# kaegi/adaptive-sph

Hardware: AMD Instinct MI355X
Metric: particle-steps/sec (whole node), 2D dam-break N=1M DFSPH; 1/2/4/8 GPUs (higher is better)
Workload: dtype f32; 1 GPU; dam_break_1m: 2D dam-break, 1024x1024 = 1 048 576 uniform-h particles, HybridDFSPH; particles=1048576, solver=HybridDFSPH, parallelism=single GPU

## Files before the change

adaptive_sph_amd/csrc/sph_api.hip:

```cpp
#include <hip/hip_runtime.h>

#include <algorithm>
#include <chrono>
#include <cmath>
#include <cstdarg>
#include <cstdio>
#include <cstdlib>
#include <cstring>
#include <string>
#include <vector>

#include "sph_context.hpp"
#include "sph_lambda.hpp"

int Profiler::find(const char* name)
{
    for (size_t i = 0; i < recs.size(); i++)
        if (recs[i].name == name) return (int)i;
    recs.push_back(Rec{name, 0, 0, {}});
    return (int)recs.size() - 1;
}
bool Profiler::wants(const char* name) const
{
    return mode == 1 || mode == 3 || mode == 4 || (mode == 2 && (step_index & 7u) == 0u && strncmp(name, "density", 7) == 0);
// ... 181 lines not shown
        for (int k = 1; k < 4; k++) {
            r.min_x = fminf(r.min_x, s[k].min_x); r.min_y = fminf(r.min_y, s[k].min_y);
            r.max_x = fmaxf(r.max_x, s[k].max_x); r.max_y = fmaxf(r.max_y, s[k].max_y);
            r.h_max = fmaxf(r.h_max, s[k].h_max); r.h_min = fminf(r.h_min, s[k].h_min);
            r.min_cfl = fminf(r.min_cfl, s[k].min_cfl);
        }
        r.pad = seq - 1u;
        *out = r;
        if (seq) {
            __threadfence_system();
            ((volatile HeaderOut*)out)->pad = seq;
        }
    }
}

__global__ __launch_bounds__(1024) void k_header_ahead(const HeaderOut* __restrict__ partials, uint32_t nparts, const SolverCtrl* __restrict__ ctrl,
                                                       HeaderOut* __restrict__ out, const DeviceStatus* __restrict__ status, SolverCtrl* __restrict__ h_ctrl,
                                                       DeviceStatus* __restrict__ h_status, uint32_t seq)
{
    if (ctrl->done == 0u) {
        if (h_ctrl && threadIdx.x == 0) {
            SolverCtrl v = *ctrl;
            v.seq = seq - 1u;
            *h_ctrl = v;
            *h_status = *status;
            __threadfence_system();
            ((volatile SolverCtrl*)h_ctrl)->seq = seq;
        }
        return;
    }
    const float INF = __uint_as_float(0x7f800000u);
    HeaderOut o{INF, INF, -INF, -INF, 0.f, INF, INF, 0};
    for (uint32_t k0 = threadIdx.x; k0 < nparts; k0 += 4096u) {
        HeaderOut q[4];
#pragma unroll
        for (uint32_t u = 0; u < 4u; u++) q[u] = partials[min(k0 + 1024u * u, nparts - 1u)];
#pragma unroll
        for (uint32_t u = 0; u < 4u; u++) {
            o.min_x = fminf(o.min_x, q[u].min_x); o.min_y = fminf(o.min_y, q[u].min_y);
            o.max_x = fmaxf(o.max_x, q[u].max_x); o.max_y = fmaxf(o.max_y, q[u].max_y);
            o.h_max = fmaxf(o.h_max, q[u].h_max); o.h_min = fminf(o.h_min, q[u].h_min);
            o.min_cfl = fminf(o.min_cfl, q[u].min_cfl);
        }
    }
    o.min_x = wave_min(o.min_x); o.min_y = wave_min(o.min_y); o.max_x = wave_max(o.max_x); o.max_y = wave_max(o.max_y);
    o.h_max = wave_max(o.h_max); o.h_min = wave_min(o.h_min); o.min_cfl = wave_min(o.min_cfl);
    __shared__ HeaderOut s[16];
    const int lane = threadIdx.x & 63, w = threadIdx.x >> 6;
    if (lane == 0) s[w] = o;
    __syncthreads();
    if (threadIdx.x == 0) {
        HeaderOut r = s[0];
        for (int k = 1; k < 16; k++) {
            r.min_x = fminf(r.min_x, s[k].min_x); r.min_y = fminf(r.min_y, s[k].min_y);
            r.max_x = fmaxf(r.max_x, s[k].max_x); r.max_y = fmaxf(r.max_y, s[k].max_y);
            r.h_max = fmaxf(r.h_max, s[k].h_max); r.h_min = fminf(r.h_min, s[k].h_min);
            r.min_cfl = fminf(r.min_cfl, s[k].min_cfl);
        }
        *out = r;
        if (h_ctrl) {
            SolverCtrl v = *ctrl;
            v.seq = seq - 1u;
            *h_ctrl = v;
            *h_status = *status;
            __threadfence_system();
            ((volatile SolverCtrl*)h_ctrl)->seq = seq;
        }
    }
}

__global__ __launch_bounds__(256) void k_pack_upload(uint32_t n, const float* __restrict__ mass, const float2* __restrict__ pos,
                                                      const float2* __restrict__ velin, float4* __restrict__ pm, float2* __restrict__ vel,
                                                      uint32_t* __restrict__ orig, float* __restrict__ lvl, float* __restrict__ lvlold,
                                                      float* __restrict__ h2_next)
{
    uint32_t i = blockIdx.x * 256 + threadIdx.x;
    if (i >= n) return;
    float2 p = pos[i];
    pm[i] = make_float4(p.x, p.y, mass[i], 0.f);
    h2_next[i] = h_from_mass(mass[i], 1.f);
    vel[i] = velin[i];
    orig[i] = i;
    lvl[i] = __uint_as_float(0x7fc00000u);
    lvlold[i] = 0.f;
// ... 193 lines not shown
    o.chain = num("SPH_CHAIN", -1);
    o.accel_generic = flag("SPH_ACCEL_GENERIC");
    o.jacobi_generic = flag("SPH_JACOBI_GENERIC");
    o.source_generic = flag("SPH_SOURCE_GENERIC");
    o.slab_general = flag("SPH_SLAB_GENERAL");
    o.slab_level_plain = flag("SPH_SLAB_LEVEL_PLAIN");
    o.level_serial = flag("SPH_LEVEL_SERIAL");
    o.level_batch8 = flag("SPH_LEVEL_BATCH8");
    o.level_queue = num("SPH_LEVEL_QUEUE", 1) != 0 ? 1 : 0;
    o.offset_lists = num("SPH_OFFSET_LISTS", 1) != 0 ? 1 : 0;
    o.no_fuse = flag("SPH_NO_FUSE");
    o.side_stream_normal = flag("SPH_SIDE_STREAM_NORMAL");
    o.tile = num("SPH_TILE", 0);
    o.ahead_build = num("SPH_AHEAD_BUILD", 1) != 0 ? 1 : 0;
    o.inc_sort = num("SPH_INC_SORT", 1);
    o.slab_paced = num("SPH_SLAB_PACED", 1) != 0 ? 1 : 0;
    o.slab_records = num("SPH_SLAB_RECORDS", 1) != 0 ? 1 : 0;
    o.side_cus = num("SPH_SIDE_CUS", 0);
    o.main_exclude = num("SPH_MAIN_EXCLUDE", 0) != 0 ? 1 : 0;
    o.ipc_fuse_max_bytes = std::max(num("SPH_IPC_FUSE_MAX_BYTES", 64 << 10), 0);
    o.ipc_copy_min_bytes = std::max(num("SPH_IPC_COPY_MIN_BYTES", 256 << 10), 0);
#else
    static const char* const lab_only[] = {"SPH_PACED", "SPH_PACE_LEAD", "SPH_PACE_PRED", "SPH_CHAIN", "SPH_ACCEL_GENERIC", "SPH_JACOBI_GENERIC", "SPH_SOURCE_GENERIC",
                                           "SPH_SLAB_GENERAL", "SPH_SLAB_LEVEL_PLAIN", "SPH_LEVEL_SERIAL", "SPH_LEVEL_BATCH8", "SPH_LEVEL_QUEUE", "SPH_OFFSET_LISTS",
                                           "SPH_NO_FUSE", "SPH_SIDE_STREAM_NORMAL", "SPH_TILE", "SPH_AHEAD_BUILD", "SPH_INC_SORT", "SPH_SLAB_PACED", "SPH_SLAB_RECORDS",
                                           "SPH_SIDE_CUS", "SPH_MAIN_EXCLUDE", "SPH_IPC_FUSE_MAX_BYTES", "SPH_IPC_COPY_MIN_BYTES"};
    static bool warned = false;
    if (!warned)
        for (const char* name : lab_only)
            if (getenv(name)) {
                fprintf(stderr, "libsph_hip: %s is a laboratory switch and is IGNORED by the product library (use SPH_HIP_LIBRARY=libsph_lab.so, scripts/README.md)\n", name);
                warned = true;
            }
#endif
    return o;
}

extern "C" int sph_create(uint64_t n_capacity, int device_id, const sph_plane* planes, int n_planes, sph_ctx** out)
{
    if (!out || n_planes < 0 || n_planes > SPH_MAX_PLANES || (n_planes > 0 && !planes)) return SPH_ERR_INVALID_ARGUMENT;
// ... 96 lines not shown
}

extern "C" void sph_destroy(sph_ctx* c)
{
    if (!c) return;
    (void)hipSetDevice(c->device);
    if (c->stream) (void)hipStreamSynchronize(c->stream);
    if (c->stream2) (void)hipStreamSynchronize(c->stream2);
    dist_release(c);
    DevBuf* all[] = {&c->pm[0], &c->pm[1], &c->vel[0], &c->vel[1], &c->orig[0], &c->orig[1], &c->lvl[0], &c->lvl[1], &c->lvlold[0],
                     &c->lvlold[1], &c->vel_tmp, &c->key[0], &c->key[1], &c->val[0], &c->val[1], &c->sort_scratch, &c->cxy, &c->cell_start,
                     &c->cs_scratch, &c->hdr_ahead_partials, &c->h2n[0], &c->h2n[1], &c->lam_prev, &c->nl, &c->nlx, &c->tile_raw, &c->tile_h, &c->tile_h_ext, &c->lvl_changed_d, &c->lvl_tmp, &c->lvl_nrm, &c->lvl_state, &c->lvl_when, &c->lvl_mark, &c->lvl_queue, &c->nloff, &c->nlh, &c->flag_surface,
                     &c->flag_insufficient, &c->con_thr, &c->con_consumed, &c->con_h, &c->flag_reduced, &c->szc[0], &c->szc[1], &c->omega, &c->stash, &c->nl_ext, &c->nlx_ext, &c->nl_ok, &c->mrho, &c->pt0, &c->pt1, &c->prec0, &c->prec1, &c->xv, &c->rho, &c->lam_sum, &c->lam_grad, &c->wall_pl, &c->wall_cnt, &c->constf, &c->aii, &c->src, &c->p0, &c->p1, &c->pacc, &c->dens_err,
                     &c->stat, &c->ncount, &c->planes_d, &c->lam_lut, &c->dlam_lut, &c->hdr_partials, &c->hdr_out, &c->ctrl, &c->status,
                     &c->n_tiles, &c->red_partials, &c->scratch, &c->split_patterns, &c->akey[0], &c->akey[1], &c->aval[0], &c->aval[1], &c->acxy, &c->acell_start, &c->pm2,
                     &c->atile_raw, &c->atile_h, &c->inc_head, &c->inc_next, &c->inc_bsum, &c->inc_movers, &c->export_d_off, &c->export_d_idx,
                     &c->cand_rec, &c->cand_cls, &c->cand_cnt, &c->cand_off, &c->cand_idx, &c->cand_scan, &c->cand_red, &c->rnd_rec, &c->rnd_keys, &c->rnd_out, &c->rnd_max, &c->rnd_prev};
    for (auto b : all) b->release();
    if (c->hdr_host) (void)hipHostFree(c->hdr_host);
    if (c->ctrl_host) (void)hipHostFree(c->ctrl_host);
    if (c->status_host) (void)hipHostFree(c->status_host);
    if (c->lvl_changed) (void)hipHostFree(c->lvl_changed);
    for (auto& e : c->ev)
        if (e) (void)hipEventDestroy(e);
    if (c->ev_sync) (void)hipEventDestroy(c->ev_sync);
    if (c->stream) (void)hipStreamDestroy(c->stream);
    if (c->stream2) (void)hipStreamDestroy(c->stream2);
    if (c->ev_fork) (void)hipEventDestroy(c->ev_fork);
    delete c;
}

// ... 814 lines not shown
    int nb = (int)((n + 255) / 256);
    if (nb > HDR_BLOCKS) nb = HDR_BLOCKS;
    if (nb < 1) nb = 1;
    hipLaunchKernelGGL(k_header, dim3(nb), dim3(256), 0, s, c->pm[c->pcur].as<float4>(), c->vel[c->cur].as<float2>(), n, rest_density, from_mass,
                       c->h2n[c->cur].as<float>(), c->hdr_partials.as<HeaderOut>(), owned);
    c->publish_seq++;
    if (c->publish_seq == 0u) c->publish_seq = 1u;
    const bool mapped = out_dev == c->hdr_host_dev;
    hipLaunchKernelGGL(k_header_final, dim3(1), dim3(256), 0, s, c->hdr_partials.as<HeaderOut>(), nb, out_dev, mapped ? c->publish_seq : 0u);
    if (mapped) {
        c->hint_word = &((volatile HeaderOut*)c->hdr_host)->pad;
        c->hint_seq = c->publish_seq;
    }
}

void launch_header_ahead(sph_ctx* c, uint32_t nblocks, HeaderOut* out_dev, bool publish)
{
    ProfScope ps(&c->prof, "header_ahead", c->stream);
    uint32_t seq = 0;
    if (publish) {
        c->publish_seq++;
        if (c->publish_seq == 0u) c->publish_seq = 1u;
        seq = c->publish_seq;
        c->publish_folded = true;
    }
    hipLaunchKernelGGL(k_header_ahead, dim3(1), dim3(1024), 0, c->stream, c->hdr_ahead_partials.as<HeaderOut>(), nblocks, c->ctrl.as<SolverCtrl>(), out_dev,
                       c->status.as<DeviceStatus>(), publish ? c->ctrl_host_dev : (SolverCtrl*)nullptr, publish ? c->status_host_dev : (DeviceStatus*)nullptr, seq);
}

void launch_publish(sph_ctx* c)
{
    if (c->publish_folded) {
        c->publish_folded = false;
        return;
    }
    c->publish_seq++;
    if (c->publish_seq == 0u) c->publish_seq = 1u;
    hipLaunchKernelGGL(k_publish, dim3(1), dim3(64), 0, c->stream, c->ctrl.as<SolverCtrl>(), c->status.as<DeviceStatus>(), c->ctrl_host_dev,
                       c->status_host_dev, c->publish_seq);
}

void launch_check_neighborhood(sph_ctx* c, const SweepArgs& a)
// ... 5 lines not shown
```

adaptive_sph_amd/csrc/sph_context.hpp:

```cpp
#pragma once

#include <hip/hip_runtime.h>

#include <chrono>
#include <cstdarg>
#include <cstdio>
#include <string>
#include <vector>

#include "sph_internal.hpp"

struct DevBuf {
    void* p = nullptr;
    size_t bytes = 0;
    hipError_t ensure(size_t need)
    {
        if (need <= bytes) return hipSuccess;
        if (p) (void)hipFree(p);
        p = nullptr;
        bytes = 0;
        size_t grow = need + need / 4 + 256;
        hipError_t e = hipMalloc(&p, grow);
        if (e == hipSuccess) bytes = grow;
        return e;
// ... 3 lines not shown
        if (p) (void)hipFree(p);
        p = nullptr;
        bytes = 0;
    }
    template <class T>
    T* as() const { return (T*)p; }
};

struct TmpBuf : DevBuf {
    TmpBuf() = default;
    TmpBuf(const TmpBuf&) = delete;
    TmpBuf& operator=(const TmpBuf&) = delete;
    ~TmpBuf() { release(); }
};

struct Options {
    int exact = 0;
    int paced = 1;
    int pace_lead = 0;
    int pace_pred = 0xffff;
    int chain = -1;
    int overlap = -1;
    int accel_generic = 0;
    int jacobi_generic = 0;
    int source_generic = 0;
    int slab_general = 0;
    int slab_level_plain = 0;
    int level_serial = 0;
    int level_batch8 = 0;
    int offset_lists = 1;
    int level_queue = 1;
// ... 108 lines not shown
        int rebalance_every = 0;
        DevBuf hist;
        uint32_t rebalances = 0;
        uint64_t stat_exchanges = 0, stat_bytes_sent = 0, stat_bytes_recv = 0, stat_allreduces = 0, stat_step0 = 0;
    } dist;

    GridP grid{};
    bool grid_valid = false;
    GridP fgrid{};
    int tile_ts = 0, tile_tsx = 0, tile_tsy = 0;
    DevBuf tile_raw, tile_h, tile_h_ext, nlx;
    DevBuf nloff, nlh;
    DevBuf akey[2], aval[2], acxy, acell_start, pm2;
    DevBuf atile_raw, atile_h;
    DevBuf inc_head, inc_next, inc_bsum, inc_movers;
    uint32_t inc_epoch = 0;
    int inc_radix_streak = 0;
    bool inc_count_valid = false;
    struct Ahead {
        bool valid = false;
        GridP g{};
        float h_max = 0.f, h_min = 0.f, rest_density = 0.f;
        int tile_ts = 0, tile_tsx = 0, tile_tsy = 0;
        uint64_t n = 0;
    } ahead;
    DevBuf hdr_ahead_partials;
    bool hdr_ahead = false;
    float hdr_ahead_rest_density = 0.f;
    DevBuf h2n[2];
    DevBuf lam_prev;
// ... 57 lines not shown
```

adaptive_sph_amd/csrc/sph_internal.hpp:

```cpp
#pragma once

#include <hip/hip_runtime.h>
#include <hip/hip_ext.h>
#include <stdint.h>

#include <string>
#include <vector>

#include "sph_device.h"
#include "sph_ffi.h"

struct Profiler {
    int mode = 0;
    uint64_t step_index = 0;
    struct Rec {
        std::string name;
        uint64_t launches = 0;
        double total_ms = 0;
        std::vector<float> samples;
    };
    struct Pending {
        int rec;
        hipEvent_t a, b;
        int slot;
// ... 47 lines not shown
    uint32_t done;
    uint32_t iters;
    uint32_t cur;
    uint32_t peer_error;
    uint32_t normal, singular, negative;
    float sum_err, max_err;
    uint32_t slot_done[2];
    uint32_t seq;
};

struct DeviceStatus {
    uint32_t error;
    uint32_t info;
};

struct CellKeyGen {
    const float4* pm;
    GridP g;
    const uint8_t* gone;
    uint32_t n_gone, gone_from;
    int clamp = 0;
};
int radix_sort_pairs(hipStream_t s, Profiler* prof, uint32_t* keyA, uint32_t* valA, uint32_t* keyB, uint32_t* valB,
                     uint32_t n, int bits, uint32_t* hist_scratch , const CellKeyGen* keygen = nullptr);
size_t radix_sort_scratch_elems(uint32_t n);
struct ReorderIO {
    const float4* pm_in;
    const float2* vel_in;
    const uint32_t* orig_in;
    const float *lvl_in, *lvlold_in;
    float4* pm_out;
    float2* vel_out;
    uint32_t* orig_out;
    float *lvl_out, *lvlold_out;
    uint32_t* cxy_out;
    const float* h2n_in;
    float* h2n_out;
    const float* lam_in;
    float* lam_prev_out;
    const uint8_t* szc_in;
    uint8_t* szc_out;
};
size_t incremental_sort_block_sums(uint32_t ncells);
void incremental_cell_sort_reorder(hipStream_t s, Profiler* prof, uint32_t n, const float4* pm_new, const IncClassifyP& q, bool classified,
                                   const uint32_t* cell_start_cur, uint32_t* key_out, uint32_t* cell_start_out, const ReorderIO& io, uint32_t* bsum, uint32_t* movers,
                                   uint32_t* movers_host);

void incremental_cell_sort_perm(hipStream_t s, Profiler* prof, uint32_t n, uint32_t n_prev, const CellKeyGen& kg, const IncClassifyP& q, const uint32_t* cell_start_cur,
                                uint32_t* key_out, uint32_t* perm_out, uint32_t* cell_start_out, uint32_t* bsum, uint32_t* movers, uint32_t* movers_host);

void launch_reorder(hipStream_t s, Profiler* prof, uint32_t n, GridP g, const uint32_t* sorted_key, const uint32_t* perm,
                    const float4* pm_in, const float2* vel_in, const uint32_t* orig_in, const float* lvl_in,
                    const float* lvlold_in, float4* pm_out, float2* vel_out, uint32_t* orig_out, float* lvl_out,
                    float* lvlold_out, uint32_t* cxy, const float* h2n_in = nullptr, float* h2n_out = nullptr,
                    const float* lam_in = nullptr, float* lam_prev_out = nullptr, void* cell_start_scratch = nullptr,
                    const uint8_t* szc_in = nullptr, uint8_t* szc_out = nullptr);
size_t cell_start_scratch_bytes();
void launch_cell_start(hipStream_t s, Profiler* prof, const uint32_t* sorted_key, uint32_t n, uint32_t ncells,
                       uint32_t* cell_start , void* scratch ,
                       bool count_zeroed = false );
void launch_tile_hmax(hipStream_t s, Profiler* prof, uint32_t n, const float4* pm, GridP g, int ts, int tsx, int tsy, uint32_t* raw,
// ... 124 lines not shown
    int center_diff;
    int plain_propagate;
    const uint8_t* edge;
    int replay_step_lists;
    const float4* pm_cell;
};
void launch_max_disp(hipStream_t s, Profiler* prof, uint32_t n, const float4* pm_old, const float4* pm_new, uint32_t* out);
void launch_tile_redilate(hipStream_t s, Profiler* prof, int tsx, int tsy, int d, const uint32_t* raw, uint32_t* out);
void launch_level_detect(hipStream_t s, Profiler* prof, const SweepArgs& a, const LevelArgs& l);
void launch_level_propagate(hipStream_t s, Profiler* prof, const SweepArgs& a, const LevelArgs& l, uint32_t t, uint32_t* changed);
void launch_fill_stash(hipStream_t s, Profiler* prof, const SweepArgs& a, const LevelArgs& l, float* stash);
void launch_level_smooth(hipStream_t s, Profiler* prof, const SweepArgs& a, const LevelArgs& l, const float4* pm_new, const float* in, float* out);
void launch_classify(hipStream_t s, Profiler* prof, uint32_t n, const float4* pm, const float* level, uint8_t* size_class, const uint8_t* owned,
                     const uint32_t* orig, DeviceStatus* status, const sph_params* p);
void launch_header_ahead(sph_ctx* c, uint32_t nblocks, HeaderOut* out_dev, bool publish = false);
void launch_iisph2_scale(hipStream_t s, Profiler* prof, const SweepArgs& a);
void launch_check_aii(hipStream_t s, Profiler* prof, const SweepArgs& a);
void launch_vel_add_pacc(hipStream_t s, Profiler* prof, const SweepArgs& a);
void launch_integrate(hipStream_t s, Profiler* prof, const SweepArgs& a, float4* pm_out, int mode);

struct EditSrc {
    uint32_t obj;
    uint32_t set_idx;
};
struct EditSet {
    uint32_t fields;
    float mass, px, py, vx, vy, h2, h2_next, lvl, lvlold;
};
struct sph_ctx;
int regather_host_order(sph_ctx* c, uint32_t n_new, const EditSrc* d_src, const EditSet* d_sets);
// ... 2 lines not shown
```

adaptive_sph_amd/csrc/sph_sort.hip:

```cpp
#include "sph_internal.hpp"

#define RS_ITEMS 32
#define RS_TILE (64 * RS_ITEMS)

template <int NB>
__device__ __forceinline__ uint64_t rs_peers(uint32_t d, bool valid)
{
    uint64_t peers = __ballot(valid);
#pragma unroll
    for (int b = 0; b < NB; b++) {
        const bool bit = (d >> b) & 1u;
        const uint64_t m = __ballot(bit);
        peers &= bit ? m : ~m;
    }
    return peers;
}

__device__ __forceinline__ uint32_t cell_key_of(const CellKeyGen& kg, uint32_t i)
{
    if (kg.gone && i < kg.n_gone && kg.gone[i] >= kg.gone_from) return kg.g.ncells;
    const float4 p = kg.pm[i];
    if (kg.clamp) return cell_key_clamped(kg.g, p.x, p.y);
    const int cx = (int)floorf(p.x / kg.g.cs) - kg.g.minx;
    const int cy = (int)floorf(p.y / kg.g.cs) - kg.g.miny;
// ... 291 lines not shown
        if (lane >= o) x += y;
    }
    if (lane == 63) ws[w] = x;
    __syncthreads();
    uint32_t run = base_s + x - own;
    for (int k = 0; k < w; k++) run += ws[k];
#pragma unroll
    for (uint32_t u = 0; u < 4u; u++) {
        if (c0 + u < ncells) cell_start[c0 + u] = run;
        run += v[u];
        if (c0 + u + 1u == ncells) cell_start[ncells] = run;
    }
    if (blockIdx.x == 0 && tid == 0) {
        *movers_host = *movers;
        *movers = 0u;
    }
}

template <bool PERM>
__global__ __launch_bounds__(256) void k_inc_place_reorder(uint32_t n, IncGrid G, const uint32_t* __restrict__ cell_start_cur, const uint32_t* __restrict__ cell_start_nxt,
                                                            const uint32_t* __restrict__ nk, const uint8_t* __restrict__ mv, const uint32_t* __restrict__ next,
                                                            const unsigned long long* __restrict__ head, uint32_t epoch, const uint32_t* __restrict__ cxy_cur,
                                                            uint32_t* __restrict__ key_out, ReorderIO io, uint32_t* __restrict__ perm_out)
{
    const uint32_t i = blockIdx.x * 256 + threadIdx.x;
    if (i >= n) return;
    const uint32_t flag = mv[i];
    if (PERM && flag == 2u) return;
    const uint32_t c = nk[i];
    const bool mover = flag != 0u;
// ... 31 lines not shown
        return;
    }
    io.pm_out[dst] = pm;
    io.vel_out[dst] = vel;
    io.orig_out[dst] = orig;
    io.lvl_out[dst] = lvl;
    io.lvlold_out[dst] = lvlold;
    if (io.h2n_in) io.h2n_out[dst] = io.h2n_in[i];
    if (io.lam_in) io.lam_prev_out[dst] = io.lam_in[i];
    if (io.szc_in) io.szc_out[dst] = io.szc_in[i];
    const uint32_t cy = c / (uint32_t)G.nxt.sx;
    io.cxy_out[dst] = (c - cy * (uint32_t)G.nxt.sx) | (cy << 16);
}

size_t incremental_sort_block_sums(uint32_t ncells) { return ((size_t)ncells + INC_CELLS - 1) / INC_CELLS; }

void incremental_cell_sort_reorder(hipStream_t s, Profiler* prof, uint32_t n, const float4* pm_new, const IncClassifyP& q, bool classified,
                                   const uint32_t* cell_start_cur, uint32_t* key_out, uint32_t* cell_start_out, const ReorderIO& io, uint32_t* bsum, uint32_t* movers,
                                   uint32_t* movers_host)
{
    const IncGrid G{q.cur, q.nxt};
    const uint32_t ncells = q.nxt.ncells, cblocks = (uint32_t)incremental_sort_block_sums(ncells);
    if (!classified) {
        ProfScope ps(prof, "inc_classify", s);
        hipLaunchKernelGGL(k_inc_classify, dim3((n + 255) / 256), dim3(256), 0, s, n, pm_new, q);
    }
    {
        ProfScope ps(prof, "inc_count", s);
        hipLaunchKernelGGL(k_inc_count, dim3(cblocks), dim3(INC_CELLS), 0, s, G, cell_start_cur, q.mv, q.next, q.head, q.epoch, cell_start_out, bsum, movers);
    }
    {
        ProfScope ps(prof, "inc_scan", s);
        hipLaunchKernelGGL(k_inc_scan, dim3(cblocks), dim3(256), 0, s, ncells, cell_start_out, bsum, movers, movers_host);
    }
    {
        ProfScope ps(prof, "inc_reorder", s);
        hipLaunchKernelGGL(k_inc_place_reorder<false>, dim3((n + 255) / 256), dim3(256), 0, s, n, G, cell_start_cur, cell_start_out, q.nk, q.mv, q.next, q.head,
                           q.epoch, q.cxy_cur, key_out, io, (uint32_t*)nullptr);
    }
}

void incremental_cell_sort_perm(hipStream_t s, Profiler* prof, uint32_t n, uint32_t n_prev, const CellKeyGen& kg, const IncClassifyP& q, const uint32_t* cell_start_cur,
                                uint32_t* key_out, uint32_t* perm_out, uint32_t* cell_start_out, uint32_t* bsum, uint32_t* movers, uint32_t* movers_host)
{
    const IncGrid G{q.cur, q.nxt};
    const uint32_t ncells = q.nxt.ncells, cblocks = (uint32_t)incremental_sort_block_sums(ncells);
    {
        ProfScope ps(prof, "inc_classify", s);
// ... 170 lines not shown
```

adaptive_sph_amd/csrc/sph_step.hip:

```cpp
#include <atomic>
#include <hip/hip_runtime.h>
#include <rccl/rccl.h>

#include <array>
#include <cmath>
#include <cstdlib>
#include <cstring>
#include <condition_variable>
#include <functional>
#include <memory>
#include <mutex>
#include <vector>

#include "sph_dist.hpp"

SweepArgs make_args(sph_ctx* c, const StepP& sp)
{
    SweepArgs a{};
    const int k = c->cur;
    a.g = c->fgrid;
    a.sp = sp;
    a.n = c->dist.on ? c->dist.n_tot : (uint32_t)c->n;
    a.exact = c->exact;
    a.cell_start = c->cell_start.as<uint32_t>();
// ... 373 lines not shown
            if (m.n) launch_jacobi_update(m.c->stream, &m.c->prof, m.a, (int)k, q.residual_density, q.max_avg_error, q.max_iters, multi);
        }
        if ((rc = exchange_and_sweep_a(G, M, q, k + 1))) return rc;
    }
    for (auto& m : M) {
        (void)hipSetDevice(m.c->device);
        SolverCtrl* hand_host = handoff ? m.c->ctrl_host_dev + 1 : nullptr;
        uint32_t* gate_out = handoff ? (uint32_t*)(m.c->ctrl.as<SolverCtrl>() + 2) : nullptr;
        if (!m.n || q.tail == 0 ) {
            if (handoff) launch_solver_handoff(m.c->stream, &m.c->prof, m.c->ctrl.as<SolverCtrl>(), hand_host, gate_out);
            continue;
        }
        launch_solver_tail(m.c->stream, &m.c->prof, m.a, q.tail, m.c->pm[m.c->pcur ^ 1].as<float4>(), -1, q.residual_density,
                           q.max_avg_error, q.max_iters, hand_host, gate_out);
        if (q.tail == 1  && source_term_on_records(m.a)) m.a.xv_ok = true;
        if (q.tail >= 2  && m.a.hdr_partials) launch_header_ahead(m.c, (m.n + 255u) / 256u, m.c->hdr_host_dev, publish_next && !multi);
    }
    return SPH_OK;
}
static void solve_stats(Member& m, const SolveQ& q, const SolverCtrl& h)
{
    m.c->pressure_cur = h.cur;
    sph_solver_stats* st = q.density_solver ? &m.st.density_solver : &m.st.div_solver;
    st->iters = h.iters;
    st->converged = 1;
    st->normal_count = h.normal;
    st->singular_count = h.singular;
    st->negative_count = h.negative;
    st->avg_error = h.normal > 0 ? h.sum_err / (float)h.normal : NAN;
    st->max_error = h.max_err;
}
// ... 118 lines not shown
        return c0->fail(SPH_ERR_INVALID_ARGUMENT, "center diff level estimation method needs density values");
    if (!p->level_estimation_after_advection && !p->use_extended_range_for_level_estimation)
        return c0->fail(SPH_ERR_INVALID_ARGUMENT, "assertion failed: simulation_params.use_extended_range_for_level_estimation");
    if (!G.multi() && c0->n == 0) return c0->fail(SPH_ERR_INVALID_ARGUMENT, "called `Option::unwrap()` on a `None` value (no particles)");
    if (!p->level_estimation_after_advection && !(p->level_estimation_range / SPH_ETA >= 2.f))
        return c0->fail(SPH_ERR_UNSUPPORTED, "level_estimation_range / 1.9 = %g < 2: the reference then steps on lists narrower than the SPH support, which this build does not cover",
                        (double)(p->level_estimation_range / SPH_ETA));
    for (auto c : G.m)
        if (c->poisoned) return c->fail(SPH_ERR_POISONED, "an earlier step failed inside the step: the particle state is undefined until sph_upload");
    *started = true;
    const bool no_records = c0->opt.accel_generic != 0;
    const bool paced = c0->opt.paced != 0 && p->max_iters <= 0x7fffu && (!G.multi() || c0->opt.slab_paced != 0);
    for (auto c : G.m) c->paced_step = paced;
    for (auto c : G.m) c->dist.overlap_env = c0->opt.overlap;
    for (auto c : G.m) c->publish_folded = false;

    const bool tev = c0->prof.mode == 1;
    for (auto& m : M) {
        (void)hipSetDevice(m.c->device);
        if (tev) (void)hipEventRecord(m.c->ev[0], m.c->stream);
    }

    std::vector<std::vector<float>> red(M.size(), std::vector<float>(8));
    int hdr_rc = SPH_OK, setup_rc = SPH_OK;
    bool slab_fused = false;
    const float slab_slack_k = (level_on && p->level_estimation_after_advection && G.multi())
                                   ? fmaxf(2.f, c0->h_max_step > 0.f ? 4.f * c0->last_dmax / c0->h_max_step : 0.f) : 0.f;
    const float halo_base_k = fmaxf(4.f, level_on ? p->level_estimation_range / SPH_ETA : 0.f);
    auto header_ready = [&](sph_ctx* c) { return h_from_mass_mode && c->hdr_ahead && c->hdr_ahead_rest_density == p->rest_density; };
    const bool ahead_usable = !G.multi() && header_ready(c0);
// ... 716 lines not shown
            if (!m.n) launch_ctrl_reset(m.c->stream, m.c->ctrl.as<SolverCtrl>(), m.a.gate);
            if (m.n) launch_source_term(m.c->stream, &m.c->prof, m.a, kind, residual_density);
        }
    };
    auto rec = [&](int e) {
        if (tev)
            for (auto& m : M) {
                (void)hipSetDevice(m.c->device);
                (void)hipEventRecord(m.c->ev[e], m.c->stream);
            }
    };
    enum { T_NONE = 0, T_VEL = 1, T_VX = 2, T_HYBRID = 3 };
    g_trace.mark(3);
    struct AheadPlan {
        bool on = false, incremental = false;
        GridP g{};
        int tile_ts = 0, tile_tsx = 0, tile_tsy = 0;
        IncClassifyP q{};
    } plan;
    auto plan_ahead_build = [&]() -> int {
        sph_ctx* c = c0;
        plan = AheadPlan{};
        if (G.multi() || !paced || !c->opt.ahead_build || !h_from_mass_mode || p->constrain_neighborhood_count || (!c->uniform_h && c->tile_ts <= 0) ||
            (c->uniform_h && c->tile_ts != 0) || c->exact || M[0].n == 0)
            return SPH_OK;
        const uint32_t n = M[0].n;
        const float cs = c->fgrid.cs;
        const int ts = c->tile_ts, margin = 2 * (ts > 0 ? ts : 1);
        GridP g{};
        g.cs = cs;
// ... 31 lines not shown
        hipStream_t s = c->stream;
        const size_t head_before = c->inc_head.bytes;
        HIPCHK(c, c->inc_head.ensure((size_t)g.ncells * 8));
        if (c->inc_head.bytes != head_before) HIPCHK(c, hipMemsetAsync(c->inc_head.p, 0, c->inc_head.bytes, s));
        HIPCHK(c, c->inc_next.ensure((size_t)c->cap * 4));
        HIPCHK(c, c->inc_bsum.ensure(incremental_sort_block_sums(g.ncells) * 4));
        if (!c->inc_movers.p) {
            HIPCHK(c, c->inc_movers.ensure(4));
            HIPCHK(c, hipMemsetAsync(c->inc_movers.p, 0, 4, s));
        }
        if (++c->inc_epoch == 0u) c->inc_epoch = 1u;
        plan.incremental = true;
        plan.q = IncClassifyP{c->fgrid, g, c->cxy.as<uint32_t>(), c->akey[1].as<uint32_t>(), c->aval[1].as<uint8_t>(), c->inc_next.as<uint32_t>(),
                              c->inc_head.as<unsigned long long>(), c->inc_epoch};
        M[0].a.inc = plan.q;
        return SPH_OK;
    };
    bool ahead_deferred = level_on;
    const std::function<int()> queue_ahead_build = [&]() -> int {
        sph_ctx* c = c0;
        if (ahead_deferred) return SPH_OK;
        c->ahead.valid = false;
        if (!plan.on) return SPH_OK;
        const uint32_t n = M[0].n;
        const GridP g = plan.g;
        hipStream_t s = c->stream;
        const int k = c->cur;
        const float4* integrated = c->pm[c->pcur ^ 1].as<float4>();
        if (plan.incremental) {
            const ReorderIO io{integrated, c->vel[k].as<float2>(), c->orig[k].as<uint32_t>(), c->lvl[k].as<float>(), c->lvlold[k].as<float>(), c->pm2.as<float4>(),
                               c->vel[k ^ 1].as<float2>(), c->orig[k ^ 1].as<uint32_t>(), c->lvl[k ^ 1].as<float>(), c->lvlold[k ^ 1].as<float>(), c->acxy.as<uint32_t>(),
                               c->h2n[k].as<float>(), c->h2n[k ^ 1].as<float>(),  nullptr, nullptr, c->szc[k].as<uint8_t>(), c->szc[k ^ 1].as<uint8_t>()};
            incremental_cell_sort_reorder(s, &c->prof, n, integrated, plan.q,  true, c->cell_start.as<uint32_t>(), c->akey[0].as<uint32_t>(),
                                          c->acell_start.as<uint32_t>(), io, c->inc_bsum.as<uint32_t>(), c->inc_movers.as<uint32_t>(),
                                          (uint32_t*)(c->ctrl_host_dev + 2) + 1);
            c->inc_count_valid = true;
        } else {
            const CellKeyGen kg{integrated, g, nullptr, 0u, (uint32_t)SC_GONE_FROM, 1};
            const int res = radix_sort_pairs(s, &c->prof, c->akey[0].as<uint32_t>(), c->aval[0].as<uint32_t>(), c->akey[1].as<uint32_t>(), c->aval[1].as<uint32_t>(), n,
                                             ilog2_ceil(g.ncells), c->sort_scratch.as<uint32_t>(), &kg);
            if (res == 1) {
                std::swap(c->akey[0], c->akey[1]);
                std::swap(c->aval[0], c->aval[1]);
            }
            launch_reorder(s, &c->prof, n, g, c->akey[0].as<uint32_t>(), c->aval[0].as<uint32_t>(), integrated, c->vel[k].as<float2>(), c->orig[k].as<uint32_t>(),
                           c->lvl[k].as<float>(), c->lvlold[k].as<float>(), c->pm2.as<float4>(), c->vel[k ^ 1].as<float2>(), c->orig[k ^ 1].as<uint32_t>(),
                           c->lvl[k ^ 1].as<float>(), c->lvlold[k ^ 1].as<float>(), c->acxy.as<uint32_t>(), c->h2n[k].as<float>(), c->h2n[k ^ 1].as<float>(),
                           c->lam_sum.as<float>(), c->lam_prev.as<float>(), c->cs_scratch.p, c->szc[k].as<uint8_t>(), c->szc[k ^ 1].as<uint8_t>());
            launch_cell_start(s, &c->prof, c->akey[0].as<uint32_t>(), n, g.ncells, c->acell_start.as<uint32_t>(), c->cs_scratch.p, true);
        }
// ... 394 lines not shown
```

Before: 2.434 billion particle-steps/s.

## Fuse incremental-sort count and scan with header-ahead reduction into one launch

Replaces the separate inc_count and inc_scan kernels with a single-pass count+scan kernel. It uses ticketed blocks and epoch-tagged decoupled lookback on per-block aggregates. The header_ahead reduction is folded into an extra block of that same launch instead of being its own kernel. This is on by default for uniform-h, single-device, non-level runs, and is meant to cut per-step launch count and serialization gaps. The cost is spin-waiting between blocks, a bounded spin timeout that could silently produce wrong offsets, and more complex state handoff.

```diff
diff --git a/adaptive_sph_amd/csrc/sph_api.hip b/adaptive_sph_amd/csrc/sph_api.hip
--- a/adaptive_sph_amd/csrc/sph_api.hip
+++ b/adaptive_sph_amd/csrc/sph_api.hip
@@ -219,60 +219,7 @@
     }
 }
 
-__global__ __launch_bounds__(1024) void k_header_ahead(const HeaderOut* __restrict__ partials, uint32_t nparts, const SolverCtrl* __restrict__ ctrl,
-                                                       HeaderOut* __restrict__ out, const DeviceStatus* __restrict__ status, SolverCtrl* __restrict__ h_ctrl,
-                                                       DeviceStatus* __restrict__ h_status, uint32_t seq)
-{
-    if (ctrl->done == 0u) {
-        if (h_ctrl && threadIdx.x == 0) {
-            SolverCtrl v = *ctrl;
-            v.seq = seq - 1u;
-            *h_ctrl = v;
-            *h_status = *status;
-            __threadfence_system();
-            ((volatile SolverCtrl*)h_ctrl)->seq = seq;
-        }
-        return;
-    }
-    const float INF = __uint_as_float(0x7f800000u);
-    HeaderOut o{INF, INF, -INF, -INF, 0.f, INF, INF, 0};
-    for (uint32_t k0 = threadIdx.x; k0 < nparts; k0 += 4096u) {
-        HeaderOut q[4];
-#pragma unroll
-        for (uint32_t u = 0; u < 4u; u++) q[u] = partials[min(k0 + 1024u * u, nparts - 1u)];
-#pragma unroll
-        for (uint32_t u = 0; u < 4u; u++) {
-            o.min_x = fminf(o.min_x, q[u].min_x); o.min_y = fminf(o.min_y, q[u].min_y);
-            o.max_x = fmaxf(o.max_x, q[u].max_x); o.max_y = fmaxf(o.max_y, q[u].max_y);
-            o.h_max = fmaxf(o.h_max, q[u].h_max); o.h_min = fminf(o.h_min, q[u].h_min);
-            o.min_cfl = fminf(o.min_cfl, q[u].min_cfl);
-        }
-    }
-    o.min_x = wave_min(o.min_x); o.min_y = wave_min(o.min_y); o.max_x = wave_max(o.max_x); o.max_y = wave_max(o.max_y);
-    o.h_max = wave_max(o.h_max); o.h_min = wave_min(o.h_min); o.min_cfl = wave_min(o.min_cfl);
-    __shared__ HeaderOut s[16];
-    const int lane = threadIdx.x & 63, w = threadIdx.x >> 6;
-    if (lane == 0) s[w] = o;
-    __syncthreads();
-    if (threadIdx.x == 0) {
-        HeaderOut r = s[0];
-        for (int k = 1; k < 16; k++) {
-            r.min_x = fminf(r.min_x, s[k].min_x); r.min_y = fminf(r.min_y, s[k].min_y);
-            r.max_x = fmaxf(r.max_x, s[k].max_x); r.max_y = fmaxf(r.max_y, s[k].max_y);
-            r.h_max = fmaxf(r.h_max, s[k].h_max); r.h_min = fminf(r.h_min, s[k].h_min);
-            r.min_cfl = fminf(r.min_cfl, s[k].min_cfl);
-        }
-        *out = r;
-        if (h_ctrl) {
-            SolverCtrl v = *ctrl;
-            v.seq = seq - 1u;
-            *h_ctrl = v;
-            *h_status = *status;
-            __threadfence_system();
-            ((volatile SolverCtrl*)h_ctrl)->seq = seq;
-        }
-    }
-}
+__global__ __launch_bounds__(1024) void k_header_ahead(HeaderAheadP a) { header_ahead_block(a); }
 
 __global__ __launch_bounds__(256) void k_pack_upload(uint32_t n, const float* __restrict__ mass, const float2* __restrict__ pos,
                                                       const float2* __restrict__ velin, float4* __restrict__ pm, float2* __restrict__ vel,
@@ -496,6 +443,7 @@
     o.tile = num("SPH_TILE", 0);
     o.ahead_build = num("SPH_AHEAD_BUILD", 1) != 0 ? 1 : 0;
     o.inc_sort = num("SPH_INC_SORT", 1);
+    o.fold = num("SPH_FOLD", SPH_FOLD_DEFAULT) & SPH_FOLD_DEFAULT;
     o.slab_paced = num("SPH_SLAB_PACED", 1) != 0 ? 1 : 0;
     o.slab_records = num("SPH_SLAB_RECORDS", 1) != 0 ? 1 : 0;
     o.side_cus = num("SPH_SIDE_CUS", 0);
@@ -505,7 +453,7 @@
 #else
     static const char* const lab_only[] = {"SPH_PACED", "SPH_PACE_LEAD", "SPH_PACE_PRED", "SPH_CHAIN", "SPH_ACCEL_GENERIC", "SPH_JACOBI_GENERIC", "SPH_SOURCE_GENERIC",
                                            "SPH_SLAB_GENERAL", "SPH_SLAB_LEVEL_PLAIN", "SPH_LEVEL_SERIAL", "SPH_LEVEL_BATCH8", "SPH_LEVEL_QUEUE", "SPH_OFFSET_LISTS",
-                                           "SPH_NO_FUSE", "SPH_SIDE_STREAM_NORMAL", "SPH_TILE", "SPH_AHEAD_BUILD", "SPH_INC_SORT", "SPH_SLAB_PACED", "SPH_SLAB_RECORDS",
+                                           "SPH_NO_FUSE", "SPH_SIDE_STREAM_NORMAL", "SPH_TILE", "SPH_AHEAD_BUILD", "SPH_INC_SORT", "SPH_FOLD", "SPH_SLAB_PACED", "SPH_SLAB_RECORDS",
                                            "SPH_SIDE_CUS", "SPH_MAIN_EXCLUDE", "SPH_IPC_FUSE_MAX_BYTES", "SPH_IPC_COPY_MIN_BYTES"};
     static bool warned = false;
     if (!warned)
@@ -632,7 +580,7 @@
                      &c->flag_insufficient, &c->con_thr, &c->con_consumed, &c->con_h, &c->flag_reduced, &c->szc[0], &c->szc[1], &c->omega, &c->stash, &c->nl_ext, &c->nlx_ext, &c->nl_ok, &c->mrho, &c->pt0, &c->pt1, &c->prec0, &c->prec1, &c->xv, &c->rho, &c->lam_sum, &c->lam_grad, &c->wall_pl, &c->wall_cnt, &c->constf, &c->aii, &c->src, &c->p0, &c->p1, &c->pacc, &c->dens_err,
                      &c->stat, &c->ncount, &c->planes_d, &c->lam_lut, &c->dlam_lut, &c->hdr_partials, &c->hdr_out, &c->ctrl, &c->status,
                      &c->n_tiles, &c->red_partials, &c->scratch, &c->split_patterns, &c->akey[0], &c->akey[1], &c->aval[0], &c->aval[1], &c->acxy, &c->acell_start, &c->pm2,
-                     &c->atile_raw, &c->atile_h, &c->inc_head, &c->inc_next, &c->inc_bsum, &c->inc_movers, &c->export_d_off, &c->export_d_idx,
+                     &c->atile_raw, &c->atile_h, &c->inc_head, &c->inc_next, &c->inc_bsum, &c->inc_movers, &c->inc_front, &c->export_d_off, &c->export_d_idx,
                      &c->cand_rec, &c->cand_cls, &c->cand_cnt, &c->cand_off, &c->cand_idx, &c->cand_scan, &c->cand_red, &c->rnd_rec, &c->rnd_keys, &c->rnd_out, &c->rnd_max, &c->rnd_prev};
     for (auto b : all) b->release();
     if (c->hdr_host) (void)hipHostFree(c->hdr_host);
@@ -1477,9 +1425,8 @@
     }
 }
 
-void launch_header_ahead(sph_ctx* c, uint32_t nblocks, HeaderOut* out_dev, bool publish)
-{
-    ProfScope ps(&c->prof, "header_ahead", c->stream);
+HeaderAheadP header_ahead_params(sph_ctx* c, uint32_t nblocks, HeaderOut* out_dev, bool publish)
+{
     uint32_t seq = 0;
     if (publish) {
         c->publish_seq++;
@@ -1487,8 +1434,14 @@
         seq = c->publish_seq;
         c->publish_folded = true;
     }
-    hipLaunchKernelGGL(k_header_ahead, dim3(1), dim3(1024), 0, c->stream, c->hdr_ahead_partials.as<HeaderOut>(), nblocks, c->ctrl.as<SolverCtrl>(), out_dev,
-                       c->status.as<DeviceStatus>(), publish ? c->ctrl_host_dev : (SolverCtrl*)nullptr, publish ? c->status_host_dev : (DeviceStatus*)nullptr, seq);
+    return HeaderAheadP{c->hdr_ahead_partials.as<HeaderOut>(), nblocks, c->ctrl.as<SolverCtrl>(), out_dev, c->status.as<DeviceStatus>(),
+                        publish ? c->ctrl_host_dev : (SolverCtrl*)nullptr, publish ? c->status_host_dev : (DeviceStatus*)nullptr, seq};
+}
+
+void launch_header_ahead(sph_ctx* c, uint32_t nblocks, HeaderOut* out_dev, bool publish)
+{
+    ProfScope ps(&c->prof, "header_ahead", c->stream);
+    hipLaunchKernelGGL(k_header_ahead, dim3(1), dim3(1024), 0, c->stream, header_ahead_params(c, nblocks, out_dev, publish));
 }
 
 void launch_publish(sph_ctx* c)
diff --git a/adaptive_sph_amd/csrc/sph_context.hpp b/adaptive_sph_amd/csrc/sph_context.hpp
--- a/adaptive_sph_amd/csrc/sph_context.hpp
+++ b/adaptive_sph_amd/csrc/sph_context.hpp
@@ -41,7 +41,12 @@
     ~TmpBuf() { release(); }
 };
 
+enum {
+    SPH_FOLD_SORT_FRONT = 4,
+    SPH_FOLD_DEFAULT = SPH_FOLD_SORT_FRONT,
+};
 struct Options {
+    int fold = SPH_FOLD_DEFAULT;
     int exact = 0;
     int paced = 1;
     int pace_lead = 0;
@@ -180,6 +185,10 @@
     DevBuf akey[2], aval[2], acxy, acell_start, pm2;
     DevBuf atile_raw, atile_h;
     DevBuf inc_head, inc_next, inc_bsum, inc_movers;
+    DevBuf inc_front;
+    bool hdr_in_sort_front = false;
+    bool hdr_front_set = false;
+    HeaderAheadP hdr_front{};
     uint32_t inc_epoch = 0;
     int inc_radix_streak = 0;
     bool inc_count_valid = false;
diff --git a/adaptive_sph_amd/csrc/sph_internal.hpp b/adaptive_sph_amd/csrc/sph_internal.hpp
--- a/adaptive_sph_amd/csrc/sph_internal.hpp
+++ b/adaptive_sph_amd/csrc/sph_internal.hpp
@@ -85,6 +85,71 @@
     uint32_t info;
 };
 
+struct HeaderAheadP {
+    const HeaderOut* partials;
+    uint32_t nparts;
+    const SolverCtrl* ctrl;
+    HeaderOut* out;
+    const DeviceStatus* status;
+    SolverCtrl* h_ctrl;
+    DeviceStatus* h_status;
+    uint32_t seq;
+};
+#ifdef __HIPCC__
+__device__ __forceinline__ void header_ahead_block(const HeaderAheadP& a)
+{
+    if (a.ctrl->done == 0u) {
+        if (a.h_ctrl && threadIdx.x == 0) {
+            SolverCtrl v = *a.ctrl;
+            v.seq = a.seq - 1u;
+            *a.h_ctrl = v;
+            *a.h_status = *a.status;
+            __threadfence_system();
+            ((volatile SolverCtrl*)a.h_ctrl)->seq = a.seq;
+        }
+        return;
+    }
+    const float INF = __uint_as_float(0x7f800000u);
+    HeaderOut o{INF, INF, -INF, -INF, 0.f, INF, INF, 0};
+    for (uint32_t k0 = threadIdx.x; k0 < a.nparts; k0 += 4096u) {
+        HeaderOut q[4];
+#pragma unroll
+        for (uint32_t u = 0; u < 4u; u++) q[u] = a.partials[min(k0 + 1024u * u, a.nparts - 1u)];
+#pragma unroll
+        for (uint32_t u = 0; u < 4u; u++) {
+            o.min_x = fminf(o.min_x, q[u].min_x); o.min_y = fminf(o.min_y, q[u].min_y);
+            o.max_x = fmaxf(o.max_x, q[u].max_x); o.max_y = fmaxf(o.max_y, q[u].max_y);
+            o.h_max = fmaxf(o.h_max, q[u].h_max); o.h_min = fminf(o.h_min, q[u].h_min);
+            o.min_cfl = fminf(o.min_cfl, q[u].min_cfl);
+        }
+    }
+    o.min_x = wave_min(o.min_x); o.min_y = wave_min(o.min_y); o.max_x = wave_max(o.max_x); o.max_y = wave_max(o.max_y);
+    o.h_max = wave_max(o.h_max); o.h_min = wave_min(o.h_min); o.min_cfl = wave_min(o.min_cfl);
+    __shared__ HeaderOut s[16];
+    const int lane = threadIdx.x & 63, w = threadIdx.x >> 6;
+    if (lane == 0) s[w] = o;
+    __syncthreads();
+    if (threadIdx.x == 0) {
+        HeaderOut r = s[0];
+        for (int k = 1; k < 16; k++) {
+            r.min_x = fminf(r.min_x, s[k].min_x); r.min_y = fminf(r.min_y, s[k].min_y);
+            r.max_x = fmaxf(r.max_x, s[k].max_x); r.max_y = fmaxf(r.max_y, s[k].max_y);
+            r.h_max = fmaxf(r.h_max, s[k].h_max); r.h_min = fminf(r.h_min, s[k].h_min);
+            r.min_cfl = fminf(r.min_cfl, s[k].min_cfl);
+        }
+        *a.out = r;
+        if (a.h_ctrl) {
+            SolverCtrl v = *a.ctrl;
+            v.seq = a.seq - 1u;
+            *a.h_ctrl = v;
+            *a.h_status = *a.status;
+            __threadfence_system();
+            ((volatile SolverCtrl*)a.h_ctrl)->seq = a.seq;
+        }
+    }
+}
+#endif
+
 struct CellKeyGen {
     const float4* pm;
     GridP g;
@@ -112,10 +177,16 @@
     const uint8_t* szc_in;
     uint8_t* szc_out;
 };
+struct IncFront {
+    unsigned long long* agg;
+    uint32_t* ticket;
+    const HeaderAheadP* hdr;
+};
 size_t incremental_sort_block_sums(uint32_t ncells);
+size_t incremental_sort_front_words(uint32_t ncells);
 void incremental_cell_sort_reorder(hipStream_t s, Profiler* prof, uint32_t n, const float4* pm_new, const IncClassifyP& q, bool classified,
                                    const uint32_t* cell_start_cur, uint32_t* key_out, uint32_t* cell_start_out, const ReorderIO& io, uint32_t* bsum, uint32_t* movers,
-                                   uint32_t* movers_host);
+                                   uint32_t* movers_host, const IncFront* front = nullptr);
 
 void incremental_cell_sort_perm(hipStream_t s, Profiler* prof, uint32_t n, uint32_t n_prev, const CellKeyGen& kg, const IncClassifyP& q, const uint32_t* cell_start_cur,
                                 uint32_t* key_out, uint32_t* perm_out, uint32_t* cell_start_out, uint32_t* bsum, uint32_t* movers, uint32_t* movers_host);
@@ -270,6 +341,7 @@
 void launch_classify(hipStream_t s, Profiler* prof, uint32_t n, const float4* pm, const float* level, uint8_t* size_class, const uint8_t* owned,
                      const uint32_t* orig, DeviceStatus* status, const sph_params* p);
 void launch_header_ahead(sph_ctx* c, uint32_t nblocks, HeaderOut* out_dev, bool publish = false);
+HeaderAheadP header_ahead_params(sph_ctx* c, uint32_t nblocks, HeaderOut* out_dev, bool publish);
 void launch_iisph2_scale(hipStream_t s, Profiler* prof, const SweepArgs& a);
 void launch_check_aii(hipStream_t s, Profiler* prof, const SweepArgs& a);
 void launch_vel_add_pacc(hipStream_t s, Profiler* prof, const SweepArgs& a);
diff --git a/adaptive_sph_amd/csrc/sph_sort.hip b/adaptive_sph_amd/csrc/sph_sort.hip
--- a/adaptive_sph_amd/csrc/sph_sort.hip
+++ b/adaptive_sph_amd/csrc/sph_sort.hip
@@ -329,6 +329,92 @@
     if (blockIdx.x == 0 && tid == 0) {
         *movers_host = *movers;
         *movers = 0u;
+    }
+}
+
+__device__ __forceinline__ uint32_t inc_front_wait(const unsigned long long* p, uint32_t epoch)
+{
+    unsigned long long v;
+    for (uint32_t spins = 0; (uint32_t)((v = __hip_atomic_load(p, __ATOMIC_RELAXED, __HIP_MEMORY_SCOPE_AGENT)) >> 32) != epoch; spins++) {
+        if (spins >= (1u << 20)) return 0u;
+        __builtin_amdgcn_s_sleep(2);
+    }
+    return (uint32_t)v;
+}
+template <bool HDR>
+__global__ __launch_bounds__(INC_CELLS) void k_inc_count_scan(IncGrid G, const uint32_t* __restrict__ cell_start_cur, const uint8_t* __restrict__ mv,
+                                                               const uint32_t* __restrict__ next, const unsigned long long* __restrict__ head, uint32_t epoch,
+                                                               uint32_t* __restrict__ cell_start, unsigned long long* agg, uint32_t* ticket, uint32_t nblocks,
+                                                               uint32_t* __restrict__ movers_host, HeaderAheadP hdr)
+{
+    if (HDR && blockIdx.x == 0u) {
+        header_ahead_block(hdr);
+        return;
+    }
+    __shared__ uint32_t ws[INC_CELLS / 64], wm[INC_CELLS / 64], wp[INC_CELLS / 64], wq[INC_CELLS / 64], s_t;
+    const uint32_t tid = threadIdx.x, lane = tid & 63u, w = tid >> 6;
+    if (tid == 0) s_t = atomicAdd(ticket, 1u);
+    __syncthreads();
+    const uint32_t t = s_t, ncells = G.nxt.ncells;
+    const uint32_t c = t * (uint32_t)INC_CELLS + tid;
+    uint32_t cnt = 0, listed = 0;
+    if (c < ncells) {
+        uint32_t b, e;
+        inc_cur_range(G, c, cell_start_cur, b, e);
+        const unsigned long long h = head[c];
+        for (uint32_t j = b; j < e; j++) cnt += mv[j] ? 0u : 1u;
+        if ((uint32_t)(h >> 32) == epoch)
+            for (uint32_t m = (uint32_t)h; m; m = next[m - 1u]) listed++;
+        cnt += listed;
+    }
+    uint32_t x = cnt, y = listed;
+#pragma unroll
+    for (int o = 1; o < 64; o <<= 1) {
+        const uint32_t u = __shfl_up(x, o, 64);
+        if (lane >= (uint32_t)o) x += u;
+    }
+    for (int o = 32; o > 0; o >>= 1) y += (uint32_t)__shfl_xor((int)y, o, 64);
+    if (lane == 63u) ws[w] = x;
+    if (lane == 0u) wm[w] = y;
+    __syncthreads();
+    uint32_t own_m = 0;
+    if (tid == 0) {
+        uint32_t sum = 0;
+        for (int k = 0; k < INC_CELLS / 64; k++) {
+            sum += ws[k];
+            own_m += wm[k];
+        }
+        __hip_atomic_store(&agg[t], ((unsigned long long)epoch << 32) | sum, __ATOMIC_RELAXED, __HIP_MEMORY_SCOPE_AGENT);
+        __hip_atomic_store(&agg[nblocks + t], ((unsigned long long)epoch << 32) | own_m, __ATOMIC_RELAXED, __HIP_MEMORY_SCOPE_AGENT);
+    }
+    const bool last = t + 1u == nblocks;
+    uint32_t pre = 0, mpre = 0;
+    for (uint32_t k = tid; k < t; k += (uint32_t)INC_CELLS) {
+        pre += inc_front_wait(&agg[k], epoch);
+        if (last) mpre += inc_front_wait(&agg[nblocks + k], epoch);
+    }
+    for (int o = 32; o > 0; o >>= 1) {
+        pre += (uint32_t)__shfl_xor((int)pre, o, 64);
+        mpre += (uint32_t)__shfl_xor((int)mpre, o, 64);
+    }
+    if (lane == 0u) {
+        wp[w] = pre;
+        wq[w] = mpre;
+    }
+    __syncthreads();
+    uint32_t run = x - cnt;
+    for (uint32_t k = 0; k < (uint32_t)(INC_CELLS / 64); k++) {
+        run += wp[k];
+        if (k < w) run += ws[k];
+    }
+    if (c < ncells) {
+        cell_start[c] = run;
+        if (c + 1u == ncells) cell_start[ncells] = run + cnt;
+    }
+    if (last && tid == 0) {
+        for (int k = 0; k < INC_CELLS / 64; k++) own_m += wq[k];
+        *movers_host = own_m;
+        atomicExch(ticket, 0u);
     }
 }
 
@@ -390,10 +476,11 @@
 }
 
 size_t incremental_sort_block_sums(uint32_t ncells) { return ((size_t)ncells + INC_CELLS - 1) / INC_CELLS; }
+size_t incremental_sort_front_words(uint32_t ncells) { return 2 * incremental_sort_block_sums(ncells); }
 
 void incremental_cell_sort_reorder(hipStream_t s, Profiler* prof, uint32_t n, const float4* pm_new, const IncClassifyP& q, bool classified,
                                    const uint32_t* cell_start_cur, uint32_t* key_out, uint32_t* cell_start_out, const ReorderIO& io, uint32_t* bsum, uint32_t* movers,
-                                   uint32_t* movers_host)
+                                   uint32_t* movers_host, const IncFront* front)
 {
     const IncGrid G{q.cur, q.nxt};
     const uint32_t ncells = q.nxt.ncells, cblocks = (uint32_t)incremental_sort_block_sums(ncells);
@@ -401,13 +488,23 @@
         ProfScope ps(prof, "inc_classify", s);
         hipLaunchKernelGGL(k_inc_classify, dim3((n + 255) / 256), dim3(256), 0, s, n, pm_new, q);
     }
-    {
-        ProfScope ps(prof, "inc_count", s);
-        hipLaunchKernelGGL(k_inc_count, dim3(cblocks), dim3(INC_CELLS), 0, s, G, cell_start_cur, q.mv, q.next, q.head, q.epoch, cell_start_out, bsum, movers);
-    }
-    {
-        ProfScope ps(prof, "inc_scan", s);
-        hipLaunchKernelGGL(k_inc_scan, dim3(cblocks), dim3(256), 0, s, ncells, cell_start_out, bsum, movers, movers_host);
+    if (front) {
+        ProfScope ps(prof, "inc_count_scan", s);
+        if (front->hdr)
+            hipLaunchKernelGGL(k_inc_count_scan<true>, dim3(cblocks + 1u), dim3(INC_CELLS), 0, s, G, cell_start_cur, q.mv, q.next, q.head, q.epoch, cell_start_out,
+                               front->agg, front->ticket, cblocks, movers_host, *front->hdr);
+        else
+            hipLaunchKernelGGL(k_inc_count_scan<false>, dim3(cblocks), dim3(INC_CELLS), 0, s, G, cell_start_cur, q.mv, q.next, q.head, q.epoch, cell_start_out,
+                               front->agg, front->ticket, cblocks, movers_host, HeaderAheadP{});
+    } else {
+        {
+            ProfScope ps(prof, "inc_count", s);
+            hipLaunchKernelGGL(k_inc_count, dim3(cblocks), dim3(INC_CELLS), 0, s, G, cell_start_cur, q.mv, q.next, q.head, q.epoch, cell_start_out, bsum, movers);
+        }
+        {
+            ProfScope ps(prof, "inc_scan", s);
+            hipLaunchKernelGGL(k_inc_scan, dim3(cblocks), dim3(256), 0, s, ncells, cell_start_out, bsum, movers, movers_host);
+        }
     }
     {
         ProfScope ps(prof, "inc_reorder", s);
diff --git a/adaptive_sph_amd/csrc/sph_step.hip b/adaptive_sph_amd/csrc/sph_step.hip
--- a/adaptive_sph_amd/csrc/sph_step.hip
+++ b/adaptive_sph_amd/csrc/sph_step.hip
@@ -411,7 +411,12 @@
         launch_solver_tail(m.c->stream, &m.c->prof, m.a, q.tail, m.c->pm[m.c->pcur ^ 1].as<float4>(), -1, q.residual_density,
                            q.max_avg_error, q.max_iters, hand_host, gate_out);
         if (q.tail == 1  && source_term_on_records(m.a)) m.a.xv_ok = true;
-        if (q.tail >= 2  && m.a.hdr_partials) launch_header_ahead(m.c, (m.n + 255u) / 256u, m.c->hdr_host_dev, publish_next && !multi);
+        if (q.tail >= 2  && m.a.hdr_partials) {
+            if (m.c->hdr_in_sort_front) {
+                m.c->hdr_front = header_ahead_params(m.c, (m.n + 255u) / 256u, m.c->hdr_host_dev, publish_next && !multi);
+                m.c->hdr_front_set = true;
+            } else launch_header_ahead(m.c, (m.n + 255u) / 256u, m.c->hdr_host_dev, publish_next && !multi);
+        }
     }
     return SPH_OK;
 }
@@ -560,6 +565,7 @@
     for (auto c : G.m) c->paced_step = paced;
     for (auto c : G.m) c->dist.overlap_env = c0->opt.overlap;
     for (auto c : G.m) c->publish_folded = false;
+    for (auto c : G.m) c->hdr_in_sort_front = c->hdr_front_set = false;
 
     const bool tev = c0->prof.mode == 1;
     for (auto& m : M) {
@@ -1306,6 +1312,7 @@
     g_trace.mark(3);
     struct AheadPlan {
         bool on = false, incremental = false;
+        bool front = false;
         GridP g{};
         int tile_ts = 0, tile_tsx = 0, tile_tsy = 0;
         IncClassifyP q{};
@@ -1367,6 +1374,13 @@
         plan.q = IncClassifyP{c->fgrid, g, c->cxy.as<uint32_t>(), c->akey[1].as<uint32_t>(), c->aval[1].as<uint8_t>(), c->inc_next.as<uint32_t>(),
                               c->inc_head.as<unsigned long long>(), c->inc_epoch};
         M[0].a.inc = plan.q;
+        if ((c->opt.fold & SPH_FOLD_SORT_FRONT) && c->uniform_h && !c->dist.on && !level_on) {
+            const size_t words = incremental_sort_front_words(g.ncells) + 1, front_before = c->inc_front.bytes;
+            HIPCHK(c, c->inc_front.ensure(words * 8));
+            if (c->inc_front.bytes != front_before) HIPCHK(c, hipMemsetAsync(c->inc_front.p, 0, c->inc_front.bytes, s));
+            plan.front = true;
+            c->hdr_in_sort_front = true;
+        }
         return SPH_OK;
     };
     bool ahead_deferred = level_on;
@@ -1384,9 +1398,12 @@
             const ReorderIO io{integrated, c->vel[k].as<float2>(), c->orig[k].as<uint32_t>(), c->lvl[k].as<float>(), c->lvlold[k].as<float>(), c->pm2.as<float4>(),
                                c->vel[k ^ 1].as<float2>(), c->orig[k ^ 1].as<uint32_t>(), c->lvl[k ^ 1].as<float>(), c->lvlold[k ^ 1].as<float>(), c->acxy.as<uint32_t>(),
                                c->h2n[k].as<float>(), c->h2n[k ^ 1].as<float>(),  nullptr, nullptr, c->szc[k].as<uint8_t>(), c->szc[k ^ 1].as<uint8_t>()};
+            const IncFront front{c->inc_front.as<unsigned long long>(), (uint32_t*)(c->inc_front.as<unsigned long long>() + (c->inc_front.bytes / 8 - 1)),
+                                 c->hdr_front_set ? &c->hdr_front : nullptr};
             incremental_cell_sort_reorder(s, &c->prof, n, integrated, plan.q,  true, c->cell_start.as<uint32_t>(), c->akey[0].as<uint32_t>(),
                                           c->acell_start.as<uint32_t>(), io, c->inc_bsum.as<uint32_t>(), c->inc_movers.as<uint32_t>(),
-                                          (uint32_t*)(c->ctrl_host_dev + 2) + 1);
+                                          (uint32_t*)(c->ctrl_host_dev + 2) + 1, plan.front ? &front : nullptr);
+            c->hdr_in_sort_front = c->hdr_front_set = false;
             c->inc_count_valid = true;
         } else {
             const CellKeyGen kg{integrated, g, nullptr, 0u, (uint32_t)SC_GONE_FROM, 1};
```

Result: faster. 2.468 billion particle-steps/s, median of 6 (+1.4%).
